# HikariTJU/LD

Hardware: AMD Instinct MI355X
Metric: images/sec (1333x800) GFocal-R50<-R101 LD train step (higher is better)
Workload: dtype f32

## Files before the change

### ld_amd/csrc/nn.hip

```cpp
#include <hip/hip_runtime.h>
#include <stdlib.h>

#include "ld_launch.h"

#include "../../include/ld_hip.h"

namespace {

__device__ __forceinline__ float wave_sum_f(float v) {
#pragma unroll
  for (int off = 32; off >= 1; off >>= 1) v += __shfl_xor(v, off);
  return v;
}
__device__ __forceinline__ double wave_sum_d(double v) {
#pragma unroll
  for (int off = 32; off >= 1; off >>= 1) v += __shfl_xor(v, off);
  return v;
}

__device__ __forceinline__ void block_sum2(double& a, double& b) {
  __shared__ double sa[4], sb[4];
  a = wave_sum_d(a);
  b = wave_sum_d(b);
  const int w = threadIdx.x >> 6;
// ... 446 lines not shown
  const float* base = x + ((size_t)n * C + (size_t)g * cpg) * lv.P + lv.off[l];
  const int per = gn_slice_len(A);
  const int beg = sp * per, end = min(A, beg + per);
  double* const slot = partial + ((size_t)ngl * kGnSplit + sp) * 2;
  double s = 0.0, q = 0.0;
  const bool al = ((uintptr_t)base % 16 == 0) && (lv.P % 4 == 0);
  const int b0 = al ? min((beg + 3) & ~3, end) : end;
  const int b1 = al ? max(end & ~3, b0) : end;
  for (int p = b0 + 4 * (int)threadIdx.x; p < b1; p += 1024) {
#pragma unroll 8
    for (int ch = 0; ch < cpg; ++ch) {
      const float4 t = *reinterpret_cast<const float4*>(base + (size_t)ch * lv.P + p);
      const double v0 = t.x, v1 = t.y, v2 = t.z, v3 = t.w;
      s += (v0 + v1) + (v2 + v3);
      q += (v0 * v0 + v1 * v1) + (v2 * v2 + v3 * v3);
    }
  }
  for (int p = beg + threadIdx.x; p < end; p += 256) {
    if (p >= b0 && p < b1) continue;
#pragma unroll 8
    for (int ch = 0; ch < cpg; ++ch) {
      const double v = (double)base[(size_t)ch * lv.P + p];
      s += v;
      q += v * v;
    }
  }
  block_sum2(s, q);
  if (threadIdx.x == 0) {
    slot[0] = s;
    slot[1] = q;
  }
}

__global__ void gn_stats_final_kernel(const double* __restrict__ partial, Levels lv,
                                      int N, int C, int G, float eps,
                                      float* __restrict__ mean,
                                      float* __restrict__ rstd) {
  const int L = lv.num_levels;
  const int ngl = blockIdx.x * blockDim.x + threadIdx.x;
  if (ngl >= N * G * L) return;
  const int l = ngl % L;
  const double total = (double)(C / G) * (lv.off[l + 1] - lv.off[l]);
  double s = 0.0, q = 0.0;
  const int nk = gn_slices(lv.off[l + 1] - lv.off[l]);
  for (int k = 0; k < nk; ++k) {
    s += partial[((size_t)ngl * kGnSplit + k) * 2 + 0];
    q += partial[((size_t)ngl * kGnSplit + k) * 2 + 1];
  }
  const double m = s / total;
  double var = q / total - m * m;
  if (var < 0.0) var = 0.0;
  mean[ngl] = (float)m;
  rstd[ngl] = (float)(1.0 / sqrt(var + (double)eps));
}

__device__ __forceinline__ float gn_affine(float in, float mu, float rs, float ga,
                                           float be) {
  return __builtin_fmaf((in - mu) * rs, ga, be);
}

__global__ __launch_bounds__(256) void gn_apply_kernel(
    const float* __restrict__ x, Levels lv, int C, int G,
    const float* __restrict__ mean, const float* __restrict__ rstd,
    const float* __restrict__ gamma, const float* __restrict__ beta, int relu,
    float* __restrict__ y) {
  const int row = blockIdx.y;
  const int c = row % C, n = row / C;
  const int p = blockIdx.x * 256 + threadIdx.x;
  if (p >= lv.P) return;
  const int l = level_of_pos(lv, p);
  const size_t o = ((size_t)n * G + c / (C / G)) * lv.num_levels + l;
  const size_t idx = (size_t)row * lv.P + p;
  float v = gn_affine(x[idx], mean[o], rstd[o], gamma[c], beta[c]);
  if (relu) v = fmaxf(v, 0.f);
  y[idx] = v;
}

__global__ __launch_bounds__(256) void gn_apply4_kernel(
    const float* __restrict__ x, Levels lv, int C, int G,
    const float* __restrict__ mean, const float* __restrict__ rstd,
    const float* __restrict__ gamma, const float* __restrict__ beta, int relu,
    float* __restrict__ y) {
  const int row = blockIdx.y;
  const int c = row % C, n = row / C;
  const int p = (blockIdx.x * 256 + threadIdx.x) * 4;
  if (p >= lv.P) return;
  const size_t ob = ((size_t)n * G + c / (C / G)) * lv.num_levels;
  const size_t idx = (size_t)row * lv.P + p;
  const float4 v = *reinterpret_cast<const float4*>(x + idx);
  const float ga = gamma[c], be = beta[c];
  const int l0 = level_of_pos(lv, p), l3 = level_of_pos(lv, p + 3);
  float in[4] = {v.x, v.y, v.z, v.w}, out[4];
  if (l0 == l3) {
    const float mu = mean[ob + l0], rs = rstd[ob + l0];
#pragma unroll
    for (int k = 0; k < 4; ++k) out[k] = gn_affine(in[k], mu, rs, ga, be);
  } else {
#pragma unroll
    for (int k = 0; k < 4; ++k) {
      const int l = level_of_pos(lv, p + k);
      out[k] = gn_affine(in[k], mean[ob + l], rstd[ob + l], ga, be);
    }
  }
  if (relu) {
#pragma unroll
    for (int k = 0; k < 4; ++k) out[k] = fmaxf(out[k], 0.f);
  }
  *reinterpret_cast<float4*>(y + idx) = make_float4(out[0], out[1], out[2], out[3]);
}

typedef float gn_floatx8 __attribute__((ext_vector_type(8)));
typedef __bf16 gn_bf16x8 __attribute__((ext_vector_type(8)));
typedef unsigned gn_uintx4 __attribute__((ext_vector_type(4)));

__device__ __forceinline__ void store_c8x4(gn_uintx4* __restrict__ dst,
                                           const float (&v)[8][4]) {
#pragma unroll
  for (int k = 0; k < 4; ++k) {
    gn_floatx8 f;
#pragma unroll
    for (int e = 0; e < 8; ++e) f[e] = v[e][k];
    dst[k] = __builtin_bit_cast(gn_uintx4, __builtin_convertvector(f, gn_bf16x8));
  }
}

__global__ __launch_bounds__(256) void bn_act_fwd_c8_kernel(
    const float* __restrict__ x, const float* __restrict__ residual,
    const float* __restrict__ scale, const float* __restrict__ shift, int C, int P,
    int relu, float* __restrict__ y, gn_uintx4* __restrict__ y_c8) {
  const int C8 = C >> 3;
  const int blk = blockIdx.y;
  const int c8 = blk % C8, n = blk / C8;
  const int p = (blockIdx.x * 256 + threadIdx.x) * 4;
  if (p >= P) return;
  float out[8][4];
#pragma unroll
  for (int e = 0; e < 8; ++e) {
    const int c = c8 * 8 + e;
    const float s = scale[c], b = shift[c];
    const size_t idx = ((size_t)n * C + c) * P + p;
    float4 v = *reinterpret_cast<const float4*>(x + idx);
// ... 289 lines not shown
  for (int e = 0; e < 8; ++e) {
    const int c = c8 * 8 + e;
    const size_t idx = ((size_t)n * C + c) * lv.P + p;
    const float ga = gamma[c];
    float be = 0.f;
    if (MASK_X) be = beta[c];
    if (!one_group) {
      gn_load_tab(tab, mean, rstd, gm, ((size_t)n * G + c / cpg) * L, L);
      gn_pick(tab, l0, mu0, rs0, f10, f20);
    }
    const float a_dy[4] = {t0[e].x, t0[e].y, t0[e].z, t0[e].w};
    const float a_x[4] = {t2[e].x, t2[e].y, t2[e].z, t2[e].w};
    float a_y[4] = {1.f, 1.f, 1.f, 1.f};
    if (!MASK_X) {
      a_y[0] = t1[e].x; a_y[1] = t1[e].y; a_y[2] = t1[e].z; a_y[3] = t1[e].w;
    }
#pragma unroll
    for (int k = 0; k < 4; ++k) {
      float mu = mu0, rs = rs0, fm1 = f10, fm2 = f20;
      if (l0 != l3) gn_pick(tab, level_of_pos(lv, p + k), mu, rs, fm1, fm2);
      float dz = a_dy[k];
      if (MASK_X) a_y[k] = gn_affine(a_x[k], mu, rs, ga, be);
      if (relu && !(a_y[k] > 0.f)) dz = 0.f;
      const float xh = (a_x[k] - mu) * rs;
      out[e][k] = rs * (ga * dz - fm1 - xh * fm2);
    }
    if (!MASK_X || dx)
      *reinterpret_cast<float4*>(dx + idx) =
          make_float4(out[e][0], out[e][1], out[e][2], out[e][3]);
  }
  store_c8x4(dx_c8 + (size_t)blk * lv.P + p, out);
}

namespace old_r5 {
__global__ __launch_bounds__(256) void gn_bwd_apply_c8_kernel(
    const float* __restrict__ dy, const float* __restrict__ y,
    const float* __restrict__ x, Levels lv, int C, int G,
    const float* __restrict__ mean, const float* __restrict__ rstd,
    const float* __restrict__ gamma, const float* __restrict__ gm, int relu,
    float* __restrict__ dx, gn_uintx4* __restrict__ dx_c8) {
  const int C8 = C >> 3;
  const int blk = blockIdx.y;
  const int c8 = blk % C8, n = blk / C8;
  const int p = (blockIdx.x * 256 + threadIdx.x) * 4;
  if (p >= lv.P) return;
  const int L = lv.num_levels;
  float out[8][4];
#pragma unroll
  for (int e = 0; e < 8; ++e) {
    const int c = c8 * 8 + e;
    const size_t ob = ((size_t)n * G + c / (C / G)) * L;
    const size_t idx = ((size_t)n * C + c) * lv.P + p;
    const float ga = gamma[c];
    const float4 t0 = *reinterpret_cast<const float4*>(dy + idx);
    const float4 t2 = *reinterpret_cast<const float4*>(x + idx);
    const float a_dy[4] = {t0.x, t0.y, t0.z, t0.w};
    const float a_x[4] = {t2.x, t2.y, t2.z, t2.w};
    float a_y[4] = {1.f, 1.f, 1.f, 1.f};
    if (relu) {
      const float4 t1 = *reinterpret_cast<const float4*>(y + idx);
      a_y[0] = t1.x; a_y[1] = t1.y; a_y[2] = t1.z; a_y[3] = t1.w;
    }
#pragma unroll
    for (int k = 0; k < 4; ++k) {
      const int l = level_of_pos(lv, p + k);
      const float mu = mean[ob + l], rs = rstd[ob + l];
      const float fm1 = gm[(ob + l) * 2 + 0], fm2 = gm[(ob + l) * 2 + 1];
      float dz = a_dy[k];
      if (relu && !(a_y[k] > 0.f)) dz = 0.f;
      const float xh = (a_x[k] - mu) * rs;
      out[e][k] = rs * (ga * dz - fm1 - xh * fm2);
    }
    *reinterpret_cast<float4*>(dx + idx) =
        make_float4(out[e][0], out[e][1], out[e][2], out[e][3]);
  }
  store_c8x4(dx_c8 + (size_t)blk * lv.P + p, out);
}

}

constexpr int kGnBwdSplit = 8;

__global__ __launch_bounds__(256) void gn_bwd_reduce_kernel(
    const float* __restrict__ dy, const float* __restrict__ y,
    const float* __restrict__ x, Levels lv, int C, int G,
    const float* __restrict__ mean, const float* __restrict__ rstd, int relu,
    double* __restrict__ sums) {
  const int L = lv.num_levels;
  const int sp = blockIdx.x % kGnBwdSplit;
  const int rl = blockIdx.x / kGnBwdSplit;
  const int l = rl % L, row = rl / L;
  const int c = row % C, n = row / C;
  const int A = lv.off[l + 1] - lv.off[l];
  const int per = max((A + kGnBwdSplit - 1) / kGnBwdSplit, 1024);
  const int beg = sp * per, end = min(A, beg + per);
  if (beg >= end) {
    if (threadIdx.x == 0) {
      sums[(size_t)blockIdx.x * 2 + 0] = 0.0;
      sums[(size_t)blockIdx.x * 2 + 1] = 0.0;
    }
    return;
  }
  const size_t o = ((size_t)n * G + c / (C / G)) * L + l;
  const float mu = mean[o], rs = rstd[o];
  const size_t base = (size_t)row * lv.P + lv.off[l];
  double s1 = 0.0, s2 = 0.0;
  for (int p = beg + threadIdx.x; p < end; p += 256) {
    float dz = dy[base + p];
    if (relu && !(y[base + p] > 0.f)) dz = 0.f;
    s1 += (double)dz;
    s2 += (double)(dz * ((x[base + p] - mu) * rs));
  }
  block_sum2(s1, s2);
// ... 50 lines not shown
    }
    const int ne = (b0 - p0) + (p1 - b1);
    if ((int)threadIdx.x < ne) {
      const int t = threadIdx.x;
      const int p = t < b0 - p0 ? p0 + t : b1 + (t - (b0 - p0));
      const size_t idx = rbase + p;
      float dz = dy[idx];
      const float xe = x[idx];
      if (relu && !((MASK_X ? gn_affine(xe, mu, rs, ga, be) : y[idx]) > 0.f)) dz = 0.f;
      s1 += (double)dz;
      s2 += (double)(dz * ((xe - mu) * rs));
    }
    block_sum2(s1, s2);
    if (threadIdx.x == 0) {
      const size_t at = ((size_t)row * L + l) * kGnBwdSplit * 2;
      sums[at + 0] = s1;
      sums[at + 1] = s2;
    }
  }
}

__global__ void gn_bwd_fold_kernel(double* __restrict__ sums, int rows_levels) {
  const int i = blockIdx.x * blockDim.x + threadIdx.x;
  if (i >= rows_levels) return;
  double s1 = 0.0, s2 = 0.0;
  for (int k = 0; k < kGnBwdSplit; ++k) {
    s1 += sums[((size_t)i * kGnBwdSplit + k) * 2 + 0];
    s2 += sums[((size_t)i * kGnBwdSplit + k) * 2 + 1];
  }
  sums[(size_t)i * kGnBwdSplit * 2 + 0] = s1;
  sums[(size_t)i * kGnBwdSplit * 2 + 1] = s2;
}

__global__ void gn_bwd_group_kernel(const double* __restrict__ sums, Levels lv, int N,
                                    int C, int G, const float* __restrict__ gamma,
                                    float* __restrict__ gm) {
  const int L = lv.num_levels;
  const int ngl = blockIdx.x * blockDim.x + threadIdx.x;
  if (ngl >= N * G * L) return;
  const int l = ngl % L, g = (ngl / L) % G, n = ngl / (L * G);
  const int cpg = C / G, A = lv.off[l + 1] - lv.off[l];
  double m1 = 0.0, m2 = 0.0;
  for (int k = 0; k < cpg; ++k) {
    const int cc = g * cpg + k;
    const size_t r = ((size_t)(n * C + cc) * L + l) * kGnBwdSplit * 2;
    m1 += (double)gamma[cc] * sums[r + 0];
    m2 += (double)gamma[cc] * sums[r + 1];
  }
  const double cnt = (double)cpg * A;
  gm[(size_t)ngl * 2 + 0] = (float)(m1 / cnt);
  gm[(size_t)ngl * 2 + 1] = (float)(m2 / cnt);
}

template <int V>
__global__ __launch_bounds__(256) void gn_bwd_apply_kernel(
    const float* __restrict__ dy, const float* __restrict__ y,
    const float* __restrict__ x, Levels lv, int C, int G,
    const float* __restrict__ mean, const float* __restrict__ rstd,
    const float* __restrict__ gamma, const float* __restrict__ gm, int relu,
    float* __restrict__ dx) {
  const int row = blockIdx.y;
  const int c = row % C, n = row / C;
  const int p = (blockIdx.x * 256 + threadIdx.x) * V;
  if (p >= lv.P) return;
  const int L = lv.num_levels, g = c / (C / G);
  const size_t idx = (size_t)row * lv.P + p;
  const float ga = gamma[c];
  GnRowTab tab;
  gn_load_tab(tab, mean, rstd, gm, ((size_t)n * G + g) * L, L);
  float a_dy[V], a_y[V], a_x[V], out[V];
  if (V == 4) {
    const float4 t0 = *reinterpret_cast<const float4*>(dy + idx);
    const float4 t2 = *reinterpret_cast<const float4*>(x + idx);
    a_dy[0] = t0.x; a_dy[1] = t0.y; a_dy[2] = t0.z; a_dy[3] = t0.w;
    a_x[0] = t2.x; a_x[1] = t2.y; a_x[2] = t2.z; a_x[3] = t2.w;
    if (relu) {
      const float4 t1 = *reinterpret_cast<const float4*>(y + idx);
      a_y[0] = t1.x; a_y[1] = t1.y; a_y[2] = t1.z; a_y[3] = t1.w;
    }
  } else {
    a_dy[0] = dy[idx];
    a_x[0] = x[idx];
    if (relu) a_y[0] = y[idx];
  }
  const int l0 = level_of_pos(lv, p), l3 = level_of_pos(lv, p + V - 1);
  float mu0, rs0, f10, f20;
  gn_pick(tab, l0, mu0, rs0, f10, f20);
#pragma unroll
  for (int k = 0; k < V; ++k) {
    float mu = mu0, rs = rs0, fm1 = f10, fm2 = f20;
    if (l0 != l3) gn_pick(tab, level_of_pos(lv, p + k), mu, rs, fm1, fm2);
    float dz = a_dy[k];
    if (relu && !(a_y[k] > 0.f)) dz = 0.f;
    const float xh = (a_x[k] - mu) * rs;
    out[k] = rs * (ga * dz - fm1 - xh * fm2);
  }
  if (V == 4)
    *reinterpret_cast<float4*>(dx + idx) = make_float4(out[0], out[1], out[2], out[3]);
  else
    dx[idx] = out[0];
}

namespace old_r5 {
template <int V>
__global__ __launch_bounds__(256) void gn_bwd_apply_kernel(
    const float* __restrict__ dy, const float* __restrict__ y,
    const float* __restrict__ x, Levels lv, int C, int G,
    const float* __restrict__ mean, const float* __restrict__ rstd,
    const float* __restrict__ gamma, const float* __restrict__ gm, int relu,
    float* __restrict__ dx) {
  const int row = blockIdx.y;
  const int c = row % C, n = row / C;
  const int p = (blockIdx.x * 256 + threadIdx.x) * V;
  if (p >= lv.P) return;
  const int L = lv.num_levels, g = c / (C / G);
  const size_t ob = ((size_t)n * G + g) * L;
  const size_t idx = (size_t)row * lv.P + p;
  const float ga = gamma[c];
  float a_dy[V], a_y[V], a_x[V], out[V];
  if (V == 4) {
    const float4 t0 = *reinterpret_cast<const float4*>(dy + idx);
    const float4 t2 = *reinterpret_cast<const float4*>(x + idx);
    a_dy[0] = t0.x; a_dy[1] = t0.y; a_dy[2] = t0.z; a_dy[3] = t0.w;
    a_x[0] = t2.x; a_x[1] = t2.y; a_x[2] = t2.z; a_x[3] = t2.w;
    if (relu) {
      const float4 t1 = *reinterpret_cast<const float4*>(y + idx);
      a_y[0] = t1.x; a_y[1] = t1.y; a_y[2] = t1.z; a_y[3] = t1.w;
    }
  } else {
    a_dy[0] = dy[idx];
    a_x[0] = x[idx];
    if (relu) a_y[0] = y[idx];
  }
#pragma unroll
  for (int k = 0; k < V; ++k) {
    const int l = level_of_pos(lv, p + k);
    const float mu = mean[ob + l], rs = rstd[ob + l];
    const float fm1 = gm[(ob + l) * 2 + 0], fm2 = gm[(ob + l) * 2 + 1];
    float dz = a_dy[k];
    if (relu && !(a_y[k] > 0.f)) dz = 0.f;
    const float xh = (a_x[k] - mu) * rs;
    out[k] = rs * (ga * dz - fm1 - xh * fm2);
  }
  if (V == 4)
    *reinterpret_cast<float4*>(dx + idx) = make_float4(out[0], out[1], out[2], out[3]);
  else
    dx[idx] = out[0];
}

}

__global__ void gn_bwd_param_kernel(const double* __restrict__ sums, int N, int C,
                                    int L, float* __restrict__ dgamma,
                                    float* __restrict__ dbeta, int accumulate) {
  const int c = blockIdx.x * blockDim.x + threadIdx.x;
  if (c >= C) return;
  double s1 = 0.0, s2 = 0.0;
  for (int n = 0; n < N; ++n)
    for (int l = 0; l < L; ++l) {
      const size_t r = ((size_t)(n * C + c) * L + l) * kGnBwdSplit * 2;
      s1 += sums[r + 0];
      s2 += sums[r + 1];
    }
  dbeta[c] = accumulate ? dbeta[c] + (float)s1 : (float)s1;
  dgamma[c] = accumulate ? dgamma[c] + (float)s2 : (float)s2;
}

__global__ __launch_bounds__(256) void maxpool3x3s2_kernel(
    const float* __restrict__ x, int rows, int H, int W, int Ho, int Wo,
    float* __restrict__ y) {
  const size_t i = (size_t)blockIdx.x * 256 + threadIdx.x;
  const size_t total = (size_t)rows * Ho * Wo;
  if (i >= total) return;
  const int wo = (int)(i % Wo);
  const size_t q = i / Wo;
  const int ho = (int)(q % Ho);
  const size_t r = q / Ho;
  const float* xp = x + r * H * W;
  float m = -INFINITY;
#pragma unroll
  for (int kh = 0; kh < 3; ++kh) {
    const int hi = ho * 2 - 1 + kh;
    if (hi < 0 || hi >= H) continue;
#pragma unroll
    for (int kw = 0; kw < 3; ++kw) {
      const int wi = wo * 2 - 1 + kw;
      if (wi < 0 || wi >= W) continue;
      m = fmaxf(m, xp[(size_t)hi * W + wi]);
    }
  }
  y[i] = m;
}

__global__ __launch_bounds__(256) void maxpool3x3s2_vec_kernel(
    const float* __restrict__ x, int rows, int H, int W, int Ho, int Wo,
    float* __restrict__ y) {
  const int half = Wo >> 1;
  const size_t i = (size_t)blockIdx.x * 256 + threadIdx.x;
// ... 653 lines not shown
                LD_STREAM, dy, y, x, scale, mean, rstd, (const double*)sums, M, N, C, P,
                relu, dx, dres);
    else
      LD_LAUNCH((bn_train_bwd_apply_kernel<false>), dim3(C, ns), dim3(256), 0,
                LD_STREAM, dy, y, x, scale, mean, rstd, (const double*)sums, M, N, C, P,
                relu, dx, dres);
  }
  return (int)hipGetLastError();
}

extern "C" int ld_bias_grad_nsplit(int N, int C, int P) {
  if (N < 1 || C < 1 || P < 1) return 0;
  return bn_splits(N, C, P);
}

extern "C" int ld_bias_grad_partial(const float* dy, int N, int C, int P, void* partial,
                                    size_t partial_bytes, ld_stream_t stream) {
  if (!dy || !partial || N < 1 || C < 1 || P < 1) return LD_EINVAL;
  const int ns = bn_splits(N, C, P);
  if (partial_bytes < (size_t)C * ns * 2 * sizeof(double)) return LD_ENOSPACE;
  LD_LAUNCH(bias_grad_partial_kernel, dim3(C, ns), dim3(256), 0, LD_STREAM, dy, N, C, P, ns,
            (double*)partial);
  return (int)hipGetLastError();
}

extern "C" int ld_bias_grad(const float* dy, int N, int C, int P, float* db,
                            int accumulate, ld_stream_t stream) {
  if (!dy || !db || N < 1 || C < 1 || P < 1) return LD_EINVAL;
  LD_LAUNCH(bias_grad_kernel, dim3(C), dim3(256), 0, LD_STREAM, dy, N, C, P,
                     db, accumulate);
  return (int)hipGetLastError();
}

extern "C" size_t ld_gn_forward_workspace_bytes(const ld_levels_t* lv, int N,
                                                int G) {
  if (check_levels(lv) != 0 || N < 1 || G < 1) return 0;
  return (size_t)N * G * lv->num_levels * kGnSplit * 2 * sizeof(double);
}

static int gn_forward_impl(const ld_levels_t* lv, const float* x, const float* gamma,
                           const float* beta, int N, int C, int G, float eps,
                           int relu, float* y, void* y_c8, float* mean, float* rstd,
                           void* workspace, size_t workspace_bytes,
                           ld_stream_t stream) {
  if (int e = check_levels(lv)) return e;
  if (!x || !gamma || !beta || (!y && !y_c8) || !mean || !rstd || N < 1 || C < 1 ||
      G < 1 || C % G)
    return LD_EINVAL;
  if (!workspace || workspace_bytes < ld_gn_forward_workspace_bytes(lv, N, G))
    return LD_ENOSPACE;
  const Levels k = make_levels(lv);
  const int ngl = N * G * k.num_levels;
  int per_ng = 0;
  for (int l = 0; l < k.num_levels; ++l) per_ng += gn_slices(k.off[l + 1] - k.off[l]);
  LD_LAUNCH(gn_stats_partial_kernel, dim3(N * G * per_ng), dim3(256), 0,
                     LD_STREAM, x, k, C, G, (double*)workspace);
  LD_LAUNCH(gn_stats_final_kernel, dim3((ngl + 255) / 256), dim3(256), 0,
                     LD_STREAM, (const double*)workspace, k, N, C, G, eps, mean,
                     rstd);
  if (y_c8) {
    if (k.P % 4 != 0 || C % 8 != 0 ||
        ((uintptr_t)x | (uintptr_t)y | (uintptr_t)y_c8) % 16 != 0)
      return LD_EUNSUPPORTED;
    LD_LAUNCH(gn_apply_c8_kernel, dim3((k.P / 4 + 255) / 256, N * (C / 8)),
                       dim3(256), 0, LD_STREAM, x, k, C, G, mean, rstd, gamma, beta,
                       relu, y, (gn_uintx4*)y_c8);
  } else if (k.P % 4 == 0 && ((uintptr_t)x | (uintptr_t)y) % 16 == 0)
    LD_LAUNCH(gn_apply4_kernel, dim3((k.P / 4 + 255) / 256, N * C),
                       dim3(256), 0, LD_STREAM, x, k, C, G, mean, rstd, gamma, beta,
                       relu, y);
  else
    LD_LAUNCH(gn_apply_kernel, dim3((k.P + 255) / 256, N * C), dim3(256), 0,
                       LD_STREAM, x, k, C, G, mean, rstd, gamma, beta, relu, y);
  return (int)hipGetLastError();
}

extern "C" int ld_gn_forward(const ld_levels_t* lv, const float* x,
                             const float* gamma, const float* beta, int N, int C,
                             int G, float eps, int relu, float* y, float* mean,
                             float* rstd, void* workspace, size_t workspace_bytes,
                             ld_stream_t stream) {
  return gn_forward_impl(lv, x, gamma, beta, N, C, G, eps, relu, y, nullptr, mean,
                         rstd, workspace, workspace_bytes, stream);
}

extern "C" int ld_gn_forward_c8(const ld_levels_t* lv, const float* x,
                                const float* gamma, const float* beta, int N, int C,
                                int G, float eps, int relu, float* y, void* y_c8,
                                float* mean, float* rstd, void* workspace,
                                size_t workspace_bytes, ld_stream_t stream) {
  if (!y_c8) return LD_EINVAL;
  return gn_forward_impl(lv, x, gamma, beta, N, C, G, eps, relu, y, y_c8, mean, rstd,
                         workspace, workspace_bytes, stream);
}

static size_t gn_bwd_sums_bytes(int L, int N, int C) {
  return (size_t)N * C * L * kGnBwdSplit * 2 * sizeof(double);
}

extern "C" size_t ld_gn_backward_workspace_bytes(const ld_levels_t* lv, int N,
                                                 int C) {
  if (check_levels(lv) != 0 || N < 1 || C < 1) return 0;
  return gn_bwd_sums_bytes(lv->num_levels, N, C) +
         (size_t)N * C * lv->num_levels * 2 * sizeof(float);
}

// ... 2 lines not shown
                            const float* mean,
                            const float* rstd, int N, int C, int G, int relu,
                            float* dx, void* dx_c8, float* dgamma, float* dbeta,
                            int accumulate, void* workspace, size_t workspace_bytes,
                            ld_stream_t stream) {
  if (int e = check_levels(lv)) return e;
  const bool lean = beta != nullptr;
  if (!dy || !x || !gamma || !mean || !rstd || (!dx && !(lean && dx_c8)) || N < 1 ||
      C < 1 || G < 1 || C % G)
    return LD_EINVAL;
  if (relu && !y && !lean) return LD_EINVAL;
  if (lean) y = dy;
  if (!workspace || workspace_bytes < ld_gn_backward_workspace_bytes(lv, N, C))
    return LD_ENOSPACE;
  const Levels k = make_levels(lv);
  double* sums = (double*)workspace;
  float* gm = (float*)((char*)workspace + gn_bwd_sums_bytes(k.num_levels, N, C));
  const int rl = N * C * k.num_levels, ngl = N * G * k.num_levels;
  const bool rowwise = k.P % 4 == 0 &&
                       ((uintptr_t)dy | (uintptr_t)x | (uintptr_t)(relu ? y : x)) % 16 == 0;
  if (lean && !rowwise) return LD_EUNSUPPORTED;
  if (rowwise && lean) {
    LD_LAUNCH(gn_bwd_reduce_row_kernel<true>, dim3(N * C), dim3(256), 0, LD_STREAM,
                       dy, y, x, k, C, G, mean, rstd, gamma, beta, relu, sums);
  } else if (rowwise) {
    LD_LAUNCH(gn_bwd_reduce_row_kernel<false>, dim3(N * C), dim3(256), 0, LD_STREAM,
                       dy, y, x, k, C, G, mean, rstd, gamma, beta, relu, sums);
  } else {
    LD_LAUNCH(gn_bwd_reduce_kernel, dim3(rl * kGnBwdSplit), dim3(256), 0,
                       LD_STREAM, dy, y, x, k, C, G, mean, rstd, relu, sums);
    LD_LAUNCH(gn_bwd_fold_kernel, dim3((rl + 255) / 256), dim3(256), 0,
                       LD_STREAM, sums, rl);
  }
  LD_LAUNCH(gn_bwd_group_kernel, dim3((ngl + 255) / 256), dim3(256), 0,
                     LD_STREAM, sums, k, N, C, G, gamma, gm);
  const bool vec = k.P % 4 == 0 &&
                   ((uintptr_t)dy | (uintptr_t)x | (uintptr_t)(dx ? dx : x) |
                    (uintptr_t)(relu ? y : x)) % 16 == 0;
  const char* old_env = getenv("LD_NN_OLD");
  const bool use_old = old_env && old_env[0] == '1';
  if (lean) {
    if (!dx_c8 || !vec || C % 8 != 0) return LD_EUNSUPPORTED;
    LD_LAUNCH(gn_bwd_apply_c8_kernel<true>,
                       dim3((k.P / 4 + 255) / 256, N * (C / 8)), dim3(256), 0,
                       LD_STREAM, dy, y, x, k, C, G, mean, rstd, gamma, beta, gm, relu,
                       dx, (gn_uintx4*)dx_c8);
  } else if (dx_c8 && use_old) {
    if (!vec || C % 8 != 0) return LD_EUNSUPPORTED;
    LD_LAUNCH(old_r5::gn_bwd_apply_c8_kernel,
                       dim3((k.P / 4 + 255) / 256, N * (C / 8)), dim3(256), 0,
                       LD_STREAM, dy, y, x, k, C, G, mean, rstd, gamma, gm, relu, dx,
                       (gn_uintx4*)dx_c8);
  } else if (use_old && vec) {
    LD_LAUNCH(old_r5::gn_bwd_apply_kernel<4>, dim3((k.P / 4 + 255) / 256, N * C),
                       dim3(256), 0, LD_STREAM, dy, y, x, k, C, G, mean, rstd, gamma,
                       gm, relu, dx);
  } else if (dx_c8) {
    if (!vec || C % 8 != 0) return LD_EUNSUPPORTED;
    LD_LAUNCH(gn_bwd_apply_c8_kernel<false>,
                       dim3((k.P / 4 + 255) / 256, N * (C / 8)), dim3(256), 0,
                       LD_STREAM, dy, y, x, k, C, G, mean, rstd, gamma, beta, gm, relu,
                       dx, (gn_uintx4*)dx_c8);
  } else if (vec)
    LD_LAUNCH(gn_bwd_apply_kernel<4>, dim3((k.P / 4 + 255) / 256, N * C),
                       dim3(256), 0, LD_STREAM, dy, y, x, k, C, G, mean, rstd, gamma,
                       gm, relu, dx);
  else
    LD_LAUNCH(gn_bwd_apply_kernel<1>, dim3((k.P + 255) / 256, N * C),
                       dim3(256), 0, LD_STREAM, dy, y, x, k, C, G, mean, rstd, gamma,
                       gm, relu, dx);
  if (dgamma && dbeta)
    LD_LAUNCH(gn_bwd_param_kernel, dim3((C + 255) / 256), dim3(256), 0,
                       LD_STREAM, sums, N, C, k.num_levels, dgamma, dbeta,
                       accumulate);
  return (int)hipGetLastError();
}

extern "C" int ld_gn_backward(const ld_levels_t* lv, const float* dy, const float* y,
                              const float* x, const float* gamma, const float* mean,
                              const float* rstd, int N, int C, int G, int relu,
                              float* dx, float* dgamma, float* dbeta, int accumulate,
                              void* workspace, size_t workspace_bytes,
                              ld_stream_t stream) {
  return gn_backward_impl(lv, dy, y, x, gamma, nullptr, mean, rstd, N, C, G, relu, dx,
                          nullptr, dgamma, dbeta, accumulate, workspace,
                          workspace_bytes, stream);
}

extern "C" int ld_gn_backward_c8(const ld_levels_t* lv, const float* dy,
                                 const float* y, const float* x, const float* gamma,
                                 const float* mean, const float* rstd, int N, int C,
                                 int G, int relu, float* dx, void* dx_c8,
                                 float* dgamma, float* dbeta, int accumulate,
                                 void* workspace, size_t workspace_bytes,
                                 ld_stream_t stream) {
  if (!dx_c8) return LD_EINVAL;
  return gn_backward_impl(lv, dy, y, x, gamma, nullptr, mean, rstd, N, C, G, relu, dx,
                          dx_c8, dgamma, dbeta, accumulate, workspace, workspace_bytes,
                          stream);
}

extern "C" int ld_gn_backward_c8_lean(const ld_levels_t* lv, const float* dy,
                                      const float* x, const float* gamma,
                                      const float* beta, const float* mean,
// ... 197 lines not shown
```

Baseline: 58.48.

## Fuse GroupNorm stat finalization and param grads into apply kernel prologues

The GroupNorm forward no longer runs a separate stats-final kernel on the non-c8 path. Each apply workgroup now reduces the partial sums itself into a shared per-level table, and one block per group writes mean and rstd. The backward non-c8 path likewise folds the group-means and dgamma/dbeta kernels into the apply kernel's prologue. The apply kernels also move to a persistent-style loop that keeps four float4 loads in flight, with a wave-uniform level lookup. This removes kernel launches and small dependent passes, at the cost of recomputing the stats in every workgroup.

```diff
diff --git a/ld_amd/csrc/nn.hip b/ld_amd/csrc/nn.hip
--- a/ld_amd/csrc/nn.hip
+++ b/ld_amd/csrc/nn.hip
@@ -502,6 +502,33 @@
   }
 }
 
+__device__ __forceinline__ void gn_stats_from_sums(double s, double q, double total,
+                                                   float eps, float& mean,
+                                                   float& rstd) {
+  const double m = s / total;
+  double var = __builtin_fma(-m, m, q / total);
+  if (var < 0.0) var = 0.0;
+  mean = (float)m;
+  rstd = (float)(1.0 / sqrt(var + (double)eps));
+}
+
+__device__ __forceinline__ void gn_stats_finish(const double* __restrict__ slot, int A,
+                                                int cpg, float eps, float& mean,
+                                                float& rstd) {
+  double s = 0.0, q = 0.0;
+  const int nk = gn_slices(A);
+  for (int k = 0; k < nk; ++k) {
+    s += slot[k * 2 + 0];
+    q += slot[k * 2 + 1];
+  }
+  gn_stats_from_sums(s, q, (double)cpg * A, eps, mean, rstd);
+}
+
+__device__ __forceinline__ double lane_value(double v, int lane) {
+  return __hiloint2double(__builtin_amdgcn_readlane(__double2hiint(v), lane),
+                          __builtin_amdgcn_readlane(__double2loint(v), lane));
+}
+
 __global__ void gn_stats_final_kernel(const double* __restrict__ partial, Levels lv,
                                       int N, int C, int G, float eps,
                                       float* __restrict__ mean,
@@ -510,18 +537,54 @@
   const int ngl = blockIdx.x * blockDim.x + threadIdx.x;
   if (ngl >= N * G * L) return;
   const int l = ngl % L;
-  const double total = (double)(C / G) * (lv.off[l + 1] - lv.off[l]);
-  double s = 0.0, q = 0.0;
-  const int nk = gn_slices(lv.off[l + 1] - lv.off[l]);
-  for (int k = 0; k < nk; ++k) {
-    s += partial[((size_t)ngl * kGnSplit + k) * 2 + 0];
-    q += partial[((size_t)ngl * kGnSplit + k) * 2 + 1];
-  }
-  const double m = s / total;
-  double var = q / total - m * m;
-  if (var < 0.0) var = 0.0;
-  mean[ngl] = (float)m;
-  rstd[ngl] = (float)(1.0 / sqrt(var + (double)eps));
+  float m, r;
+  gn_stats_finish(partial + (size_t)ngl * kGnSplit * 2, lv.off[l + 1] - lv.off[l],
+                  C / G, eps, m, r);
+  mean[ngl] = m;
+  rstd[ngl] = r;
+}
+
+__device__ __forceinline__ int level_size(const Levels& lv, int l) {
+  int A = 0;
+#pragma unroll
+  for (int i = 0; i < LD_MAX_LEVELS; ++i)
+    if (i == l) A = lv.off[i + 1] - lv.off[i];
+  return A;
+}
+
+__device__ __forceinline__ bool wave_straddles(int l0, int l3) {
+  return __builtin_amdgcn_ballot_w64(l0 != l3) != 0;
+}
+
+__device__ __forceinline__ void gn_stats_prologue(
+    const double* __restrict__ partial, const Levels& lv, int cpg, int ng, float eps,
+    bool store, float* __restrict__ mean, float* __restrict__ rstd, float2* stat) {
+  static_assert(kGnSplit <= 64, "one lane per partial pair");
+  const int L = lv.num_levels, lane = threadIdx.x & 63;
+  for (int l = threadIdx.x >> 6; l < L; l += 4) {
+    const int ngl = ng * L + l, A = level_size(lv, l), nk = gn_slices(A);
+    const double* slot = partial + (size_t)ngl * kGnSplit * 2;
+    double ps = 0.0, pq = 0.0;
+    if (lane < nk) {
+      ps = slot[lane * 2 + 0];
+      pq = slot[lane * 2 + 1];
+    }
+    double s = 0.0, q = 0.0;
+    for (int k = 0; k < nk; ++k) {
+      s += lane_value(ps, k);
+      q += lane_value(pq, k);
+    }
+    float m, r;
+    gn_stats_from_sums(s, q, (double)cpg * A, eps, m, r);
+    if (lane == 0) {
+      stat[l] = make_float2(m, r);
+      if (store) {
+        mean[ngl] = m;
+        rstd[ngl] = r;
+      }
+    }
+  }
+  __syncthreads();
 }
 
 __device__ __forceinline__ float gn_affine(float in, float mu, float rs, float ga,
@@ -529,6 +592,7 @@
   return __builtin_fmaf((in - mu) * rs, ga, be);
 }
 
+namespace parent {
 __global__ __launch_bounds__(256) void gn_apply_kernel(
     const float* __restrict__ x, Levels lv, int C, int G,
     const float* __restrict__ mean, const float* __restrict__ rstd,
@@ -577,6 +641,79 @@
     for (int k = 0; k < 4; ++k) out[k] = fmaxf(out[k], 0.f);
   }
   *reinterpret_cast<float4*>(y + idx) = make_float4(out[0], out[1], out[2], out[3]);
+}
+}
+
+constexpr int kGnDepth = 4;
+
+__device__ __forceinline__ float4 gn_affine4(const float4 v, int p, const Levels& lv,
+                                             const float2* stat, float ga, float be,
+                                             int relu) {
+  const int l0 = level_of_pos(lv, p), l3 = level_of_pos(lv, p + 3);
+  const float in[4] = {v.x, v.y, v.z, v.w};
+  float2 st[4];
+  st[0] = st[1] = st[2] = st[3] = stat[l0];
+  if (wave_straddles(l0, l3)) {
+#pragma unroll
+    for (int k = 1; k < 4; ++k) st[k] = stat[level_of_pos(lv, p + k)];
+  }
+  float out[4];
+#pragma unroll
+  for (int k = 0; k < 4; ++k) {
+    out[k] = gn_affine(in[k], st[k].x, st[k].y, ga, be);
+    if (relu) out[k] = fmaxf(out[k], 0.f);
+  }
+  return make_float4(out[0], out[1], out[2], out[3]);
+}
+
+__global__ __launch_bounds__(256) void gn_apply4_kernel(
+    const float* __restrict__ x, Levels lv, int C, int G,
+    const double* __restrict__ partial, float eps, const float* __restrict__ gamma,
+    const float* __restrict__ beta, int relu, int per4, float* __restrict__ y,
+    float* __restrict__ mean, float* __restrict__ rstd) {
+  const int row = blockIdx.y;
+  const int c = row % C, n = row / C;
+  const int cpg = C / G, g = c / cpg;
+  __shared__ float2 stat[LD_MAX_LEVELS];
+  gn_stats_prologue(partial, lv, cpg, n * G + g, eps, blockIdx.x == 0 && c == g * cpg,
+                    mean, rstd, stat);
+  const float ga = gamma[c], be = beta[c];
+  const int q0 = blockIdx.x * per4, q1 = min(lv.P >> 2, q0 + per4);
+  const float4* x4 = reinterpret_cast<const float4*>(x + (size_t)row * lv.P);
+  float4* y4 = reinterpret_cast<float4*>(y + (size_t)row * lv.P);
+  for (int qb = q0 + (int)threadIdx.x; qb < q1; qb += kGnDepth * 256) {
+    float4 v[kGnDepth];
+#pragma unroll
+    for (int u = 0; u < kGnDepth; ++u) {
+      const int q = qb + u * 256;
+      v[u] = x4[q < q1 ? q : qb];
+    }
+#pragma unroll
+    for (int u = 0; u < kGnDepth; ++u) {
+      const int q = qb + u * 256;
+      if (q < q1) y4[q] = gn_affine4(v[u], q * 4, lv, stat, ga, be, relu);
+    }
+  }
+}
+
+__global__ __launch_bounds__(256) void gn_apply_kernel(
+    const float* __restrict__ x, Levels lv, int C, int G,
+    const double* __restrict__ partial, float eps, const float* __restrict__ gamma,
+    const float* __restrict__ beta, int relu, float* __restrict__ y,
+    float* __restrict__ mean, float* __restrict__ rstd) {
+  const int row = blockIdx.y;
+  const int c = row % C, n = row / C;
+  const int cpg = C / G, g = c / cpg;
+  __shared__ float2 stat[LD_MAX_LEVELS];
+  gn_stats_prologue(partial, lv, cpg, n * G + g, eps, blockIdx.x == 0 && c == g * cpg,
+                    mean, rstd, stat);
+  const int p = blockIdx.x * 256 + threadIdx.x;
+  if (p >= lv.P) return;
+  const float2 st = stat[level_of_pos(lv, p)];
+  const size_t idx = (size_t)row * lv.P + p;
+  float v = gn_affine(x[idx], st.x, st.y, gamma[c], beta[c]);
+  if (relu) v = fmaxf(v, 0.f);
+  y[idx] = v;
 }
 
 typedef float gn_floatx8 __attribute__((ext_vector_type(8)));
@@ -932,53 +1069,6 @@
   store_c8x4(dx_c8 + (size_t)blk * lv.P + p, out);
 }
 
-namespace old_r5 {
-__global__ __launch_bounds__(256) void gn_bwd_apply_c8_kernel(
-    const float* __restrict__ dy, const float* __restrict__ y,
-    const float* __restrict__ x, Levels lv, int C, int G,
-    const float* __restrict__ mean, const float* __restrict__ rstd,
-    const float* __restrict__ gamma, const float* __restrict__ gm, int relu,
-    float* __restrict__ dx, gn_uintx4* __restrict__ dx_c8) {
-  const int C8 = C >> 3;
-  const int blk = blockIdx.y;
-  const int c8 = blk % C8, n = blk / C8;
-  const int p = (blockIdx.x * 256 + threadIdx.x) * 4;
-  if (p >= lv.P) return;
-  const int L = lv.num_levels;
-  float out[8][4];
-#pragma unroll
-  for (int e = 0; e < 8; ++e) {
-    const int c = c8 * 8 + e;
-    const size_t ob = ((size_t)n * G + c / (C / G)) * L;
-    const size_t idx = ((size_t)n * C + c) * lv.P + p;
-    const float ga = gamma[c];
-    const float4 t0 = *reinterpret_cast<const float4*>(dy + idx);
-    const float4 t2 = *reinterpret_cast<const float4*>(x + idx);
-    const float a_dy[4] = {t0.x, t0.y, t0.z, t0.w};
-    const float a_x[4] = {t2.x, t2.y, t2.z, t2.w};
-    float a_y[4] = {1.f, 1.f, 1.f, 1.f};
-    if (relu) {
-      const float4 t1 = *reinterpret_cast<const float4*>(y + idx);
-      a_y[0] = t1.x; a_y[1] = t1.y; a_y[2] = t1.z; a_y[3] = t1.w;
-    }
-#pragma unroll
-    for (int k = 0; k < 4; ++k) {
-      const int l = level_of_pos(lv, p + k);
-      const float mu = mean[ob + l], rs = rstd[ob + l];
-      const float fm1 = gm[(ob + l) * 2 + 0], fm2 = gm[(ob + l) * 2 + 1];
-      float dz = a_dy[k];
-      if (relu && !(a_y[k] > 0.f)) dz = 0.f;
-      const float xh = (a_x[k] - mu) * rs;
-      out[e][k] = rs * (ga * dz - fm1 - xh * fm2);
-    }
-    *reinterpret_cast<float4*>(dx + idx) =
-        make_float4(out[e][0], out[e][1], out[e][2], out[e][3]);
-  }
-  store_c8x4(dx_c8 + (size_t)blk * lv.P + p, out);
-}
-
-}
-
 constexpr int kGnBwdSplit = 8;
 
 __global__ __launch_bounds__(256) void gn_bwd_reduce_kernel(
@@ -1095,6 +1185,38 @@
   sums[(size_t)i * kGnBwdSplit * 2 + 1] = s2;
 }
 
+__device__ __forceinline__ void gn_group_means(const double* __restrict__ sums, int n,
+                                               int C, int L, int l, int g, int cpg,
+                                               int A, const float* __restrict__ gamma,
+                                               float& f1, float& f2) {
+  double m1 = 0.0, m2 = 0.0;
+  for (int k = 0; k < cpg; ++k) {
+    const int cc = g * cpg + k;
+    const size_t r = ((size_t)(n * C + cc) * L + l) * kGnBwdSplit * 2;
+    m1 = __builtin_fma((double)gamma[cc], sums[r + 0], m1);
+    m2 = __builtin_fma((double)gamma[cc], sums[r + 1], m2);
+  }
+  const double cnt = (double)cpg * A;
+  f1 = (float)(m1 / cnt);
+  f2 = (float)(m2 / cnt);
+}
+
+__device__ __forceinline__ void gn_param_sums(const double* __restrict__ sums, int N,
+                                              int C, int L, int c,
+                                              float* __restrict__ dgamma,
+                                              float* __restrict__ dbeta,
+                                              int accumulate) {
+  double s1 = 0.0, s2 = 0.0;
+  for (int n = 0; n < N; ++n)
+    for (int l = 0; l < L; ++l) {
+      const size_t r = ((size_t)(n * C + c) * L + l) * kGnBwdSplit * 2;
+      s1 += sums[r + 0];
+      s2 += sums[r + 1];
+    }
+  dbeta[c] = accumulate ? dbeta[c] + (float)s1 : (float)s1;
+  dgamma[c] = accumulate ? dgamma[c] + (float)s2 : (float)s2;
+}
+
 __global__ void gn_bwd_group_kernel(const double* __restrict__ sums, Levels lv, int N,
                                     int C, int G, const float* __restrict__ gamma,
                                     float* __restrict__ gm) {
@@ -1102,19 +1224,13 @@
   const int ngl = blockIdx.x * blockDim.x + threadIdx.x;
   if (ngl >= N * G * L) return;
   const int l = ngl % L, g = (ngl / L) % G, n = ngl / (L * G);
-  const int cpg = C / G, A = lv.off[l + 1] - lv.off[l];
-  double m1 = 0.0, m2 = 0.0;
-  for (int k = 0; k < cpg; ++k) {
-    const int cc = g * cpg + k;
-    const size_t r = ((size_t)(n * C + cc) * L + l) * kGnBwdSplit * 2;
-    m1 += (double)gamma[cc] * sums[r + 0];
-    m2 += (double)gamma[cc] * sums[r + 1];
-  }
-  const double cnt = (double)cpg * A;
-  gm[(size_t)ngl * 2 + 0] = (float)(m1 / cnt);
-  gm[(size_t)ngl * 2 + 1] = (float)(m2 / cnt);
-}
-
+  float f1, f2;
+  gn_group_means(sums, n, C, L, l, g, C / G, lv.off[l + 1] - lv.off[l], gamma, f1, f2);
+  gm[(size_t)ngl * 2 + 0] = f1;
+  gm[(size_t)ngl * 2 + 1] = f2;
+}
+
+namespace parent {
 template <int V>
 __global__ __launch_bounds__(256) void gn_bwd_apply_kernel(
     const float* __restrict__ dy, const float* __restrict__ y,
@@ -1163,54 +1279,142 @@
   else
     dx[idx] = out[0];
 }
-
-namespace old_r5 {
-template <int V>
+}
+
+__device__ __forceinline__ void gn_bwd_prologue(
+    const double* __restrict__ sums, const Levels& lv, int N, int C, int G, int n,
+    int c, const float* __restrict__ mean, const float* __restrict__ rstd,
+    const float* __restrict__ gamma, float* __restrict__ dgamma,
+    float* __restrict__ dbeta, int accumulate, float4* stat) {
+  const int L = lv.num_levels, lane = threadIdx.x & 63, w = threadIdx.x >> 6;
+  const int cpg = C / G, g = c / cpg;
+  for (int l = w; l < L; l += 4) {
+    double m1 = 0.0, m2 = 0.0;
+    for (int base = 0; base < cpg; base += 64) {
+      double gk = 0.0, a1 = 0.0, a2 = 0.0;
+      if (base + lane < cpg) {
+        const int cc = g * cpg + base + lane;
+        const size_t r = ((size_t)(n * C + cc) * L + l) * kGnBwdSplit * 2;
+        gk = (double)gamma[cc];
+        a1 = sums[r + 0];
+        a2 = sums[r + 1];
+      }
+      const int cnt = min(64, cpg - base);
+      for (int k = 0; k < cnt; ++k) {
+        const double gv = lane_value(gk, k);
+        m1 = __builtin_fma(gv, lane_value(a1, k), m1);
+        m2 = __builtin_fma(gv, lane_value(a2, k), m2);
+      }
+    }
+    if (lane == 0) {
+      const size_t o = ((size_t)n * G + g) * L + l;
+      const double cnt = (double)cpg * level_size(lv, l);
+      stat[l] = make_float4(mean[o], rstd[o], (float)(m1 / cnt), (float)(m2 / cnt));
+    }
+  }
+  if (dgamma && n == 0 && blockIdx.x == 0 && w == 3) {
+    double s1 = 0.0, s2 = 0.0;
+    for (int base = 0; base < N * L; base += 64) {
+      double a1 = 0.0, a2 = 0.0;
+      const int e = base + lane;
+      if (e < N * L) {
+        const size_t r = ((size_t)((e / L) * C + c) * L + e % L) * kGnBwdSplit * 2;
+        a1 = sums[r + 0];
+        a2 = sums[r + 1];
+      }
+      const int cnt = min(64, N * L - base);
+      for (int k = 0; k < cnt; ++k) {
+        s1 += lane_value(a1, k);
+        s2 += lane_value(a2, k);
+      }
+    }
+    if (lane == 0) {
+      dbeta[c] = accumulate ? dbeta[c] + (float)s1 : (float)s1;
+      dgamma[c] = accumulate ? dgamma[c] + (float)s2 : (float)s2;
+    }
+  }
+  __syncthreads();
+}
+
+__device__ __forceinline__ float gn_dx(float dy, float y, float x, int relu, float mu,
+                                       float rs, float ga, float fm1, float fm2) {
+  float dz = dy;
+  if (relu && !(y > 0.f)) dz = 0.f;
+  const float xh = (x - mu) * rs;
+  return rs * __builtin_fmaf(-xh, fm2, __builtin_fmaf(ga, dz, -fm1));
+}
+
+__global__ __launch_bounds__(256) void gn_bwd_apply4_kernel(
+    const float* __restrict__ dy, const float* __restrict__ y,
+    const float* __restrict__ x, Levels lv, int N, int C, int G,
+    const float* __restrict__ mean, const float* __restrict__ rstd,
+    const float* __restrict__ gamma, const double* __restrict__ sums, int relu,
+    int per4, float* __restrict__ dx, float* __restrict__ dgamma,
+    float* __restrict__ dbeta, int accumulate) {
+  const int row = blockIdx.y;
+  const int c = row % C, n = row / C;
+  __shared__ float4 stat[LD_MAX_LEVELS];
+  gn_bwd_prologue(sums, lv, N, C, G, n, c, mean, rstd, gamma, dgamma, dbeta, accumulate,
+                  stat);
+  const float ga = gamma[c];
+  const int q0 = blockIdx.x * per4, q1 = min(lv.P >> 2, q0 + per4);
+  const size_t rbase = (size_t)row * lv.P;
+  const float4* g4 = reinterpret_cast<const float4*>(dy + rbase);
+  const float4* x4 = reinterpret_cast<const float4*>(x + rbase);
+  const float4* y4 = reinterpret_cast<const float4*>((relu ? y : dy) + rbase);
+  float4* o4 = reinterpret_cast<float4*>(dx + rbase);
+  for (int qb = q0 + (int)threadIdx.x; qb < q1; qb += kGnDepth * 256) {
+    float4 tg[kGnDepth], ty[kGnDepth], tx[kGnDepth];
+#pragma unroll
+    for (int u = 0; u < kGnDepth; ++u) {
+      const int q = qb + u * 256;
+      const int qs = q < q1 ? q : qb;
+      tg[u] = g4[qs];
+      ty[u] = y4[qs];
+      tx[u] = x4[qs];
+    }
+#pragma unroll
+    for (int u = 0; u < kGnDepth; ++u) {
+      const int q = qb + u * 256, p = q * 4;
+      if (q >= q1) continue;
+      const float a_dy[4] = {tg[u].x, tg[u].y, tg[u].z, tg[u].w};
+      const float a_y[4] = {ty[u].x, ty[u].y, ty[u].z, ty[u].w};
+      const float a_x[4] = {tx[u].x, tx[u].y, tx[u].z, tx[u].w};
+      const int l0 = level_of_pos(lv, p), l3 = level_of_pos(lv, p + 3);
+      float4 st[4];
+      st[0] = st[1] = st[2] = st[3] = stat[l0];
+      if (wave_straddles(l0, l3)) {
+#pragma unroll
+        for (int k = 1; k < 4; ++k) st[k] = stat[level_of_pos(lv, p + k)];
+      }
+      float out[4];
+#pragma unroll
+      for (int k = 0; k < 4; ++k)
+        out[k] = gn_dx(a_dy[k], a_y[k], a_x[k], relu, st[k].x, st[k].y, ga, st[k].z,
+                       st[k].w);
+      o4[q] = make_float4(out[0], out[1], out[2], out[3]);
+    }
+  }
+}
+
 __global__ __launch_bounds__(256) void gn_bwd_apply_kernel(
     const float* __restrict__ dy, const float* __restrict__ y,
-    const float* __restrict__ x, Levels lv, int C, int G,
+    const float* __restrict__ x, Levels lv, int N, int C, int G,
     const float* __restrict__ mean, const float* __restrict__ rstd,
-    const float* __restrict__ gamma, const float* __restrict__ gm, int relu,
-    float* __restrict__ dx) {
+    const float* __restrict__ gamma, const double* __restrict__ sums, int relu,
+    float* __restrict__ dx, float* __restrict__ dgamma, float* __restrict__ dbeta,
+    int accumulate) {
   const int row = blockIdx.y;
   const int c = row % C, n = row / C;
-  const int p = (blockIdx.x * 256 + threadIdx.x) * V;
+  __shared__ float4 stat[LD_MAX_LEVELS];
+  gn_bwd_prologue(sums, lv, N, C, G, n, c, mean, rstd, gamma, dgamma, dbeta, accumulate,
+                  stat);
+  const int p = blockIdx.x * 256 + threadIdx.x;
   if (p >= lv.P) return;
-  const int L = lv.num_levels, g = c / (C / G);
-  const size_t ob = ((size_t)n * G + g) * L;
   const size_t idx = (size_t)row * lv.P + p;
-  const float ga = gamma[c];
-  float a_dy[V], a_y[V], a_x[V], out[V];
-  if (V == 4) {
-    const float4 t0 = *reinterpret_cast<const float4*>(dy + idx);
-    const float4 t2 = *reinterpret_cast<const float4*>(x + idx);
-    a_dy[0] = t0.x; a_dy[1] = t0.y; a_dy[2] = t0.z; a_dy[3] = t0.w;
-    a_x[0] = t2.x; a_x[1] = t2.y; a_x[2] = t2.z; a_x[3] = t2.w;
-    if (relu) {
-      const float4 t1 = *reinterpret_cast<const float4*>(y + idx);
-      a_y[0] = t1.x; a_y[1] = t1.y; a_y[2] = t1.z; a_y[3] = t1.w;
-    }
-  } else {
-    a_dy[0] = dy[idx];
-    a_x[0] = x[idx];
-    if (relu) a_y[0] = y[idx];
-  }
-#pragma unroll
-  for (int k = 0; k < V; ++k) {
-    const int l = level_of_pos(lv, p + k);
-    const float mu = mean[ob + l], rs = rstd[ob + l];
-    const float fm1 = gm[(ob + l) * 2 + 0], fm2 = gm[(ob + l) * 2 + 1];
-    float dz = a_dy[k];
-    if (relu && !(a_y[k] > 0.f)) dz = 0.f;
-    const float xh = (a_x[k] - mu) * rs;
-    out[k] = rs * (ga * dz - fm1 - xh * fm2);
-  }
-  if (V == 4)
-    *reinterpret_cast<float4*>(dx + idx) = make_float4(out[0], out[1], out[2], out[3]);
-  else
-    dx[idx] = out[0];
-}
-
+  const float4 st = stat[level_of_pos(lv, p)];
+  dx[idx] = gn_dx(dy[idx], relu ? y[idx] : 1.f, x[idx], relu, st.x, st.y, gamma[c], st.z,
+                  st.w);
 }
 
 __global__ void gn_bwd_param_kernel(const double* __restrict__ sums, int N, int C,
@@ -1218,15 +1422,7 @@
                                     float* __restrict__ dbeta, int accumulate) {
   const int c = blockIdx.x * blockDim.x + threadIdx.x;
   if (c >= C) return;
-  double s1 = 0.0, s2 = 0.0;
-  for (int n = 0; n < N; ++n)
-    for (int l = 0; l < L; ++l) {
-      const size_t r = ((size_t)(n * C + c) * L + l) * kGnBwdSplit * 2;
-      s1 += sums[r + 0];
-      s2 += sums[r + 1];
-    }
-  dbeta[c] = accumulate ? dbeta[c] + (float)s1 : (float)s1;
-  dgamma[c] = accumulate ? dgamma[c] + (float)s2 : (float)s2;
+  gn_param_sums(sums, N, C, L, c, dgamma, dbeta, accumulate);
 }
 
 __global__ __launch_bounds__(256) void maxpool3x3s2_kernel(
@@ -1946,6 +2142,18 @@
   return (int)hipGetLastError();
 }
 
+static bool gn_use_parent() {
+  const char* e = getenv("LD_NN_OLD");
+  return e && e[0] == '1';
+}
+
+constexpr int kGnApplyWgs = 1024;
+static int gn_apply_per4(int P4, int rows) {
+  const int chunks = kGnApplyWgs / rows > 1 ? kGnApplyWgs / rows : 1;
+  const int per4 = ((P4 + chunks - 1) / chunks + 255) & ~255;
+  return per4 > 2 * kGnDepth * 256 ? per4 : 2 * kGnDepth * 256;
+}
+
 extern "C" size_t ld_gn_forward_workspace_bytes(const ld_levels_t* lv, int N,
                                                 int G) {
   if (check_levels(lv) != 0 || N < 1 || G < 1) return 0;
@@ -1969,9 +2177,12 @@
   for (int l = 0; l < k.num_levels; ++l) per_ng += gn_slices(k.off[l + 1] - k.off[l]);
   LD_LAUNCH(gn_stats_partial_kernel, dim3(N * G * per_ng), dim3(256), 0,
                      LD_STREAM, x, k, C, G, (double*)workspace);
-  LD_LAUNCH(gn_stats_final_kernel, dim3((ngl + 255) / 256), dim3(256), 0,
-                     LD_STREAM, (const double*)workspace, k, N, C, G, eps, mean,
-                     rstd);
+  const bool use_old = gn_use_parent();
+  if (y_c8 || use_old)
+    LD_LAUNCH(gn_stats_final_kernel, dim3((ngl + 255) / 256), dim3(256), 0,
+                       LD_STREAM, (const double*)workspace, k, N, C, G, eps, mean,
+                       rstd);
+  const bool vec = k.P % 4 == 0 && ((uintptr_t)x | (uintptr_t)y) % 16 == 0;
   if (y_c8) {
     if (k.P % 4 != 0 || C % 8 != 0 ||
         ((uintptr_t)x | (uintptr_t)y | (uintptr_t)y_c8) % 16 != 0)
@@ -1979,13 +2190,22 @@
     LD_LAUNCH(gn_apply_c8_kernel, dim3((k.P / 4 + 255) / 256, N * (C / 8)),
                        dim3(256), 0, LD_STREAM, x, k, C, G, mean, rstd, gamma, beta,
                        relu, y, (gn_uintx4*)y_c8);
-  } else if (k.P % 4 == 0 && ((uintptr_t)x | (uintptr_t)y) % 16 == 0)
-    LD_LAUNCH(gn_apply4_kernel, dim3((k.P / 4 + 255) / 256, N * C),
+  } else if (use_old && vec)
+    LD_LAUNCH(parent::gn_apply4_kernel, dim3((k.P / 4 + 255) / 256, N * C),
                        dim3(256), 0, LD_STREAM, x, k, C, G, mean, rstd, gamma, beta,
                        relu, y);
-  else
+  else if (use_old)
+    LD_LAUNCH(parent::gn_apply_kernel, dim3((k.P + 255) / 256, N * C), dim3(256), 0,
+                       LD_STREAM, x, k, C, G, mean, rstd, gamma, beta, relu, y);
+  else if (vec) {
+    const int per4 = gn_apply_per4(k.P / 4, N * C);
+    LD_LAUNCH(gn_apply4_kernel, dim3((k.P / 4 + per4 - 1) / per4, N * C), dim3(256), 0,
+                       LD_STREAM, x, k, C, G, (const double*)workspace, eps, gamma,
+                       beta, relu, per4, y, mean, rstd);
+  } else
     LD_LAUNCH(gn_apply_kernel, dim3((k.P + 255) / 256, N * C), dim3(256), 0,
-                       LD_STREAM, x, k, C, G, mean, rstd, gamma, beta, relu, y);
+                       LD_STREAM, x, k, C, G, (const double*)workspace, eps, gamma,
+                       beta, relu, y, mean, rstd);
   return (int)hipGetLastError();
 }
 
@@ -2054,44 +2274,44 @@
     LD_LAUNCH(gn_bwd_fold_kernel, dim3((rl + 255) / 256), dim3(256), 0,
                        LD_STREAM, sums, rl);
   }
-  LD_LAUNCH(gn_bwd_group_kernel, dim3((ngl + 255) / 256), dim3(256), 0,
-                     LD_STREAM, sums, k, N, C, G, gamma, gm);
   const bool vec = k.P % 4 == 0 &&
                    ((uintptr_t)dy | (uintptr_t)x | (uintptr_t)(dx ? dx : x) |
                     (uintptr_t)(relu ? y : x)) % 16 == 0;
-  const char* old_env = getenv("LD_NN_OLD");
-  const bool use_old = old_env && old_env[0] == '1';
-  if (lean) {
+  const bool fused = !lean && !dx_c8 && !gn_use_parent();
+  if (!dgamma || !dbeta) dgamma = dbeta = nullptr;
+  if (!fused)
+    LD_LAUNCH(gn_bwd_group_kernel, dim3((ngl + 255) / 256), dim3(256), 0,
+                       LD_STREAM, sums, k, N, C, G, gamma, gm);
+  if (lean || dx_c8) {
     if (!dx_c8 || !vec || C % 8 != 0) return LD_EUNSUPPORTED;
-    LD_LAUNCH(gn_bwd_apply_c8_kernel<true>,
-                       dim3((k.P / 4 + 255) / 256, N * (C / 8)), dim3(256), 0,
-                       LD_STREAM, dy, y, x, k, C, G, mean, rstd, gamma, beta, gm, relu,
-                       dx, (gn_uintx4*)dx_c8);
-  } else if (dx_c8 && use_old) {
-    if (!vec || C % 8 != 0) return LD_EUNSUPPORTED;
-    LD_LAUNCH(old_r5::gn_bwd_apply_c8_kernel,
-                       dim3((k.P / 4 + 255) / 256, N * (C / 8)), dim3(256), 0,
-                       LD_STREAM, dy, y, x, k, C, G, mean, rstd, gamma, gm, relu, dx,
-                       (gn_uintx4*)dx_c8);
-  } else if (use_old && vec) {
-    LD_LAUNCH(old_r5::gn_bwd_apply_kernel<4>, dim3((k.P / 4 + 255) / 256, N * C),
+    if (lean)
+      LD_LAUNCH(gn_bwd_apply_c8_kernel<true>,
+                         dim3((k.P / 4 + 255) / 256, N * (C / 8)), dim3(256), 0,
+                         LD_STREAM, dy, y, x, k, C, G, mean, rstd, gamma, beta, gm,
+                         relu, dx, (gn_uintx4*)dx_c8);
+    else
+      LD_LAUNCH(gn_bwd_apply_c8_kernel<false>,
+                         dim3((k.P / 4 + 255) / 256, N * (C / 8)), dim3(256), 0,
+                         LD_STREAM, dy, y, x, k, C, G, mean, rstd, gamma, beta, gm,
+                         relu, dx, (gn_uintx4*)dx_c8);
+  } else if (!fused && vec)
+    LD_LAUNCH(parent::gn_bwd_apply_kernel<4>, dim3((k.P / 4 + 255) / 256, N * C),
                        dim3(256), 0, LD_STREAM, dy, y, x, k, C, G, mean, rstd, gamma,
                        gm, relu, dx);
-  } else if (dx_c8) {
-    if (!vec || C % 8 != 0) return LD_EUNSUPPORTED;
-    LD_LAUNCH(gn_bwd_apply_c8_kernel<false>,
-                       dim3((k.P / 4 + 255) / 256, N * (C / 8)), dim3(256), 0,
-                       LD_STREAM, dy, y, x, k, C, G, mean, rstd, gamma, beta, gm, relu,
-                       dx, (gn_uintx4*)dx_c8);
-  } else if (vec)
-    LD_LAUNCH(gn_bwd_apply_kernel<4>, dim3((k.P / 4 + 255) / 256, N * C),
+  else if (!fused)
+    LD_LAUNCH(parent::gn_bwd_apply_kernel<1>, dim3((k.P + 255) / 256, N * C),
                        dim3(256), 0, LD_STREAM, dy, y, x, k, C, G, mean, rstd, gamma,
                        gm, relu, dx);
-  else
-    LD_LAUNCH(gn_bwd_apply_kernel<1>, dim3((k.P + 255) / 256, N * C),
-                       dim3(256), 0, LD_STREAM, dy, y, x, k, C, G, mean, rstd, gamma,
-                       gm, relu, dx);
-  if (dgamma && dbeta)
+  else if (vec) {
+    const int per4 = gn_apply_per4(k.P / 4, N * C);
+    LD_LAUNCH(gn_bwd_apply4_kernel, dim3((k.P / 4 + per4 - 1) / per4, N * C),
+                       dim3(256), 0, LD_STREAM, dy, y, x, k, N, C, G, mean, rstd, gamma,
+                       (const double*)sums, relu, per4, dx, dgamma, dbeta, accumulate);
+  } else
+    LD_LAUNCH(gn_bwd_apply_kernel, dim3((k.P + 255) / 256, N * C), dim3(256), 0,
+                       LD_STREAM, dy, y, x, k, N, C, G, mean, rstd, gamma,
+                       (const double*)sums, relu, dx, dgamma, dbeta, accumulate);
+  if (!fused && dgamma)
     LD_LAUNCH(gn_bwd_param_kernel, dim3((C + 255) / 256), dim3(256), 0,
                        LD_STREAM, sums, N, C, k.num_levels, dgamma, dbeta,
                        accumulate);
```

Result: no change. 58.74, median of 6 (+0.4%).
